# danieleschmidt/spin-torque-rl-gym

Hardware: AMD Instinct MI355X
Metric: env_steps_per_sec (higher is better)
Workload: dtype f64

## Files before the change

### spin-torque-rl-gym_amd/csrc/stg_kernels.hpp

```cpp
#pragma once
#include "../../include/spintorque_hip.h"
#include "stg_launch_plan.hpp"
#include "stg_physics.hpp"

#include <hip/hip_runtime.h>

#include <type_traits>

using namespace stg;

struct alignas(16) EnvRec {
    double m[3];
    double tgt[3];
    double etot;
    uint32_t stepw;
    uint32_t rng;
};
static_assert(sizeof(EnvRec) == 64, "state record size");
constexpr uint32_t STG_DONE_BIT = 0x80000000u;

struct StateView {
    EnvRec* rec;
};

// ... 400 lines not shown
        } else {
            write_obs(a.final_obs + ko * 12 * N, N, i, m, tgt, row, a.c, step, etot, J, T);
        }
    }
    if (do_reset) {
        device_reset_draw(a.c.seed, env_id, rng, a.c, true, true, m, tgt);
        etot = 0.0; step = 0; done = false;
        J = 0.0; T = 0.0;
    }
    if (wr) {
        if (a.records) {
            write_record((char*)a.obs + ko * N * STG_RECORD_BYTES, i, m, tgt, row, a.c, step, etot, J, T, (float)reward,
                         (is_success ? 1u : 0u) | (truncated ? 0x100u : 0u) | ((uint32_t)st << 16));
        } else {
            write_obs(a.obs + ko * 12 * N, N, i, m, tgt, row, a.c, step, etot, J, T);
            a.reward[ko * N + i] = (float)reward;
            a.term[ko * N + i] = is_success ? 1 : 0;
            a.trunc[ko * N + i] = truncated ? 1 : 0;
        }
        if (a.reward64) a.reward64[ko * N + i] = reward;
        if (a.energy) a.energy[ko * N + i] = energy;
        if (a.status) a.status[ko * N + i] = st;
    }
}

constexpr int REFILL_STRIPES = 64;
constexpr int REFILL_CURSOR_STRIDE = 16;

template <bool THERMAL, bool MULTI, bool AXIS_Z, typename AT, bool IDS>
__device__ __forceinline__ void refill_wave(const StepArgs& a, int64_t w, int64_t nw, int64_t blk0, int64_t nblk_q, int lane, const double* s_tab,
                                            unsigned long long& c_steps, unsigned long long& c_sub, unsigned long long& c_noop) {
    const int64_t N = a.N;
    const int64_t tiles = (N + TILE_ENVS - 1) / TILE_ENVS;
    if (w == 0 && lane < REFILL_STRIPES) a.refill_cursor_next[lane * REFILL_CURSOR_STRIDE] = 0ull;
    const AT* act = (const AT*)a.actions;
    const Recorder norec{};
    const LlgsEnergyK noek{};
    const Dp5Tab tb = make_dp5_tab();
    InlineNormals ns;

    int64_t i = 0, o = 0;
    bool has_env = false;
    double J = 0.0, T = 0.0;
    V3 e_tgt{0.0, 0.0, 1.0};
    double e_etot = 0.0;
    int32_t e_step = 0;
    uint32_t e_rng = 0;
    bool e_skip = false;
    const double* row = a.ctab;
    LlgsK k = load_llgs(row);
    LlgsLane L;
    L.active = false; L.idle = true; L.rejected = false; L.attempts = 0; L.npts = 0;
    L.y = L.f = L.m0 = V3{0.0, 0.0, 1.0};
    L.t = L.T = L.h_abs = L.min_step = L.bJ = L.bpJ = 0.0;
    V3 out_m{0.0, 0.0, 1.0};

    auto take = [&](int64_t p, bool want) {
        const int64_t idx = blk0 + (p >> 6);
        const bool valid_blk = want && (p >> 6) < nblk_q;
        const int64_t slot = (valid_blk ? refill_slot_base(idx, tiles) : 0) + (p & 63);
        const bool valid = valid_blk && slot < N;
        if (!valid) return;
        if constexpr (IDS) {
            o = a.perm ? (int64_t)a.perm[slot] : slot;
            const uint32_t id = a.ids[o];
            if ((int64_t)id >= a.n_state) { write_bad_id(a, o); return; }
            i = (int64_t)id;
        } else {
            i = a.perm ? (int64_t)a.perm[slot] : slot;
        }
        V3 m;
        bool done;
        load_state(a.s, i, m, e_tgt, e_etot, e_step, e_rng, done);
        const uint32_t rng = e_rng;
        if (a.perm) {
            typedef typename std::conditional<std::is_same<AT, double>::value, double2, float2>::type AT2;
            const AT2 aa = ((const AT2*)a.act_sorted)[slot];
            parse_action<AT>(aa.x, aa.y, a.c.max_current, a.c.max_duration, J, T);
        } else {
            const int64_t p = IDS ? o : i;
            parse_action<AT>(act[p], act[N + p], a.c.max_current, a.c.max_duration, J, T);
        }
        if (MULTI) {
            const int c = (int)a.cls[i];
            row = s_tab + (c < a.ncls ? c : 0) * C_COUNT;
            k = load_llgs(row);
        }
        const RngKey rk{a.c.seed, (uint64_t)(a.env_id0 + i), rng};
        e_skip = a.c.skip_done && done;
        llgs_lane_begin<THERMAL, false, AXIS_Z>(L, out_m, m, J, T, k, row[C_BETA], row[C_BETAP], a.c.rtol, a.c.atol, a.c.max_step, rk,
                                                norec, noek, ns, !e_skip);
        has_env = true;
    };
    auto finish = [&]() {
        const SolveOut so = llgs_lane_finish<false>(L, out_m, norec, noek, ns);
        V3 m = L.m0, tgt = e_tgt;
        double etot = e_etot;
        int32_t step = e_step;
        uint32_t rng = e_rng;
        bool done = e_skip;
        env_step_tail(a, IDS ? o : i, 0, true, true, !e_skip, row, (uint64_t)(a.env_id0 + i), m, tgt, etot, step, rng, done, J, T, so, c_steps, c_sub, c_noop);
        store_state(a.s, i, m, tgt, etot, step, rng, done);
        has_env = false;
        L.active = false;
    };

    take(w * 64 + lane, true);
    const int64_t n_rest = nblk_q > nw ? nblk_q - nw : 0;
    static_assert(REFILL_STRIPES == 64, "one lane per stripe when a wavefront looks for a stripe that still has entries");
    int stripe = (int)(w % REFILL_STRIPES);
    bool queue_open = true;
    int64_t loc_q = 0, loc_end = 0;
    int loc_stripe = 0, full_streak = 0;
    bool more = n_rest > 0;
    const int check = a.refill_check > 0 ? a.refill_check : 1;
    for (;;) {
        LlgsMasks M = llgs_masks_open(L);
        for (int c = 0; c < check; ++c) {
            llgs_lane_gate<false>(L, M, (int32_t)a.c.max_attempts);
            if (M.active == 0ull) break;
            V3 z2{0.0, 0.0, 0.0}, z3{0.0, 0.0, 0.0};
            llgs_lane_attempt<THERMAL, false, AXIS_Z, false>(L, M, 0, out_m, k, tb, a.c.rtol, a.c.atol, a.c.max_step, norec, noek, ns, z2, z3);
        }
        llgs_masks_close(L, M);
        const bool fin = has_env && !L.active;
        if (__ballot(fin) != 0ull || (more && __ballot(!has_env) != 0ull)) {
            if (fin) finish();
            const unsigned long long takers = __ballot(!has_env);
            if (more && takers != 0ull) {
                const int n_take = (int)__builtin_popcountll(takers), first = (int)__builtin_ctzll(takers);
                const int rank = (int)__builtin_popcountll(takers & ((1ull << lane) - 1ull));
                const int64_t avail = loc_end - loc_q;
                const int need_new = n_take > avail ? (int)(n_take - avail) : 0;
                int64_t new_q = 0;
                const int new_stripe = stripe;
                if (need_new > 0 && queue_open) {
                    const int reserve = (takers == ~0ull && full_streak >= 1) ? 4 * 64 : need_new;
                    unsigned long long base = 0;
                    if (lane == first) base = atomicAdd(a.refill_cursor + stripe * REFILL_CURSOR_STRIDE, (unsigned long long)reserve);
                    base = (unsigned long long)__shfl((long long)base, first);
                    new_q = (int64_t)base;
                    const int64_t stripe_end = ((n_rest - stripe + REFILL_STRIPES - 1) / REFILL_STRIPES) * 64;
                    int64_t new_end = new_q + reserve;
                    if (new_end >= stripe_end) {
                        new_end = stripe_end;
                        const int64_t end_l = ((n_rest - lane + REFILL_STRIPES - 1) / REFILL_STRIPES) * 64;
                        const unsigned long long cur_l = __hip_atomic_load(a.refill_cursor + lane * REFILL_CURSOR_STRIDE, __ATOMIC_RELAXED, __HIP_MEMORY_SCOPE_AGENT);
                        unsigned long long open_s = __ballot((int64_t)cur_l < end_l);
                        open_s &= ~(1ull << stripe);
                        if (open_s == 0ull) queue_open = false;
                        else {
                            const unsigned long long after = stripe == 63 ? 0ull : (open_s >> (stripe + 1)) << (stripe + 1);
                            stripe = (int)__builtin_ctzll(after != 0ull ? after : open_s);
                        }
                    }
                    const bool from_old = rank < avail;
                    const int64_t q = from_old ? loc_q + rank : new_q + (rank - avail);
                    const int st = from_old ? loc_stripe : new_stripe;
                    const int64_t r = (q >> 6) * REFILL_STRIPES + st;
                    take((nw + r) * 64 + (q & 63), !has_env && r < n_rest && (from_old || q < new_end));
                    loc_q = new_q + need_new < new_end ? new_q + need_new : new_end;
                    loc_end = new_end;
                    loc_stripe = new_stripe;
                } else {
                    const int64_t q = loc_q + rank;
                    const int64_t r = (q >> 6) * REFILL_STRIPES + loc_stripe;
                    take((nw + r) * 64 + (q & 63), !has_env && q < loc_end && r < n_rest);
                    loc_q = loc_q + n_take < loc_end ? loc_q + n_take : loc_end;
                }
                more = queue_open || loc_q < loc_end;
                full_streak = takers == ~0ull ? full_streak + 1 : 0;
            }
        }
        if (__ballot(has_env) == 0ull && !more) break;
    }
// ... 230 lines not shown
```

### spin-torque-rl-gym_amd/csrc/stg_physics.hpp

```cpp
#pragma once

#include <hip/hip_runtime.h>
#include <stdint.h>
#include <type_traits>

#include "stg_minstep.hpp"

namespace stg {

enum ClassConst : int {
    C_EX = 0, C_EY, C_EZ,
    C_HK,
    C_MS,
    C_ALPHA,
    C_GEFF,
    C_POL,
    C_MSV,
    C_HS_SIMPLE,
    C_RX, C_RY, C_RZ,
    C_DX, C_DY, C_DZ,
    C_HEX,
    C_BETA, C_BETAP,
    C_GAMMA,
    C_HS_LLGS,
// ... 29 lines not shown
    r[C_HS_SIMPLE] = sqrt(2 * p.damping * 1.38e-23 * temperature / (mu0 * p.ms * p.volume * gamma));
    r[C_RX] = p.easy_axis[0]; r[C_RY] = p.easy_axis[1]; r[C_RZ] = p.easy_axis[2];
    r[C_DX] = -p.ms * p.demag[0]; r[C_DY] = -p.ms * p.demag[1]; r[C_DZ] = -p.ms * p.demag[2];
    r[C_HEX] = p.a_ex > 0 ? (2 * p.a_ex / (mu0 * p.ms)) * 0.1 : 0.0;
    r[C_BETA] = p.polarization * gamma / (2 * p.ms * p.volume);
    r[C_BETAP] = 0.1 * r[C_BETA];
    r[C_GAMMA] = gamma;
    r[C_HS_LLGS] = sqrt(2 * p.damping * 1.380649e-23 * temperature / (gamma * mu0 * p.ms * p.volume));
    r[C_KUV] = p.ku * p.volume;
    r[C_EDEMAG] = 0.5 * mu0 * (p.ms * p.ms) * p.volume;
    r[C_NX] = p.demag[0]; r[C_NY] = p.demag[1]; r[C_NZ] = p.demag[2];
    r[C_AREA] = p.area; r[C_RP] = p.r_p; r[C_RAP] = p.r_ap;
    r[C_TMR] = (p.r_ap - p.r_p) / p.r_p;
    const double rn = sqrt((p.ref_m[0] * p.ref_m[0] + p.ref_m[1] * p.ref_m[1]) + p.ref_m[2] * p.ref_m[2]);
    r[C_REFX] = p.ref_m[0] / rn; r[C_REFY] = p.ref_m[1] / rn; r[C_REFZ] = p.ref_m[2] / rn;
    r[C_RSERIES] = p.r_series;
    r[C_DEVTYPE] = (double)p.dev_type;
    r[C_VALID] = p.params_valid ? 1.0 : 0.0;
    r[C_SOT_DL] = p.sot_tau_dl; r[C_SOT_FL] = p.sot_tau_fl;
    r[C_SIGX] = p.sot_sigma[0]; r[C_SIGY] = p.sot_sigma[1]; r[C_SIGZ] = p.sot_sigma[2];
    r[C_KU] = p.ku;
    r[C_VCMA_XI] = p.vcma_xi;
    r[C_VCMA_TD2] = p.vcma_td * p.vcma_td;
    r[C_VCMA_VBD] = p.vcma_vbd;
    r[C_MU0MS] = mu0 * p.ms;
}

struct V3 {
    double x, y, z;
};

__device__ __forceinline__ double mul_x(double a, double b) {
#pragma clang fp contract(off)
    const double r = a * b;
    return r;
}
__device__ __forceinline__ double add_x(double a, double b) {
#pragma clang fp contract(off)
    const double r = a + b;
    return r;
}
__device__ __forceinline__ double sub_x(double a, double b) {
#pragma clang fp contract(off)
    const double r = a - b;
    return r;
}

__device__ __forceinline__ double rsqrt_fast(double s) {
    const double y = __builtin_amdgcn_rsq(s);
    const double e = __builtin_fma(-(s * y), y, 1.0);
    return __builtin_fma(y * e, __builtin_fma(0.375, e, 0.5), y);
}

__device__ __forceinline__ double vgpr_const(double c) {
    asm volatile("" : "+v"(c));
    return c;
}

__device__ __forceinline__ double fmax_abs(double a, double b) {
    double r;
    asm("v_max_f64 %0, |%1|, |%2|" : "=v"(r) : "v"(a), "v"(b));
    return r;
}

__device__ __forceinline__ void commit_step(unsigned long long mask, double& d0, double s0, double& d1, double s1, double& d2, double s2,
                                            double& d3, double s3, double& d4, double s4, double& d5, double s5, double& d6, double s6,
                                            double& min_step, double& h, double unit) {
    unsigned long long saved;
    int e;
    asm("s_and_saveexec_b64 %[sv], %[m]\n\t"
        "v_mov_b64 %[d0], %[s0]\n\t"
        "v_mov_b64 %[d1], %[s1]\n\t"
        "v_mov_b64 %[d2], %[s2]\n\t"
        "v_mov_b64 %[d3], %[s3]\n\t"
        "v_mov_b64 %[d4], %[s4]\n\t"
        "v_mov_b64 %[d5], %[s5]\n\t"
        "v_mov_b64 %[d6], %[s6]\n\t"
        "v_frexp_exp_i32_f64 %[e], %[s0]\n\t"
        "v_max_i32 %[e], %[fl], %[e]\n\t"
        "v_ldexp_f64 %[ms], %[u], %[e]\n\t"
        "v_max_f64 %[h], %[h], %[ms]\n\t"
        "s_mov_b64 exec, %[sv]"
        : [d0] "+v"(d0), [d1] "+v"(d1), [d2] "+v"(d2), [d3] "+v"(d3), [d4] "+v"(d4), [d5] "+v"(d5), [d6] "+v"(d6), [ms] "+v"(min_step),
          [h] "+v"(h), [e] "=&v"(e), [sv] "=&s"(saved)
        : [s0] "v"(s0), [s1] "v"(s1), [s2] "v"(s2), [s3] "v"(s3), [s4] "v"(s4), [s5] "v"(s5), [s6] "v"(s6), [u] "v"(unit), [m] "s"(mask),
          [fl] "n"(MIN_STEP_EXP_FLOOR)
        : "scc");
}

__device__ __forceinline__ double rcp_fast(double x) {
    const double y = __builtin_amdgcn_rcp(x);
    return __builtin_fma(y, __builtin_fma(-x, y, 1.0), y);
}

__device__ __forceinline__ double inv_tenth_root(double e2) {
    const double y = (double)__builtin_amdgcn_exp2f(-0.1f * __builtin_amdgcn_logf((float)e2));
    const double y2 = y * y, y4 = y2 * y2, y8 = y4 * y4;
    const double e = __builtin_fma(-e2, y8 * y2, 1.0);
    return __builtin_fma(y * e, __builtin_fma(0.055, e, 0.1), y);
}

__device__ __forceinline__ double fifth_root(double x) {
    int e;
    const double mant = frexp(x, &e);
    const double t = -0.2 * ((double)e + (double)__builtin_amdgcn_logf((float)mant));
    const double ti = rint(t);
    double r = ldexp((double)__builtin_amdgcn_exp2f((float)(t - ti)), (int)ti);
    const double r2 = r * r, r4 = r2 * r2;
    const double err = __builtin_fma(-x, r4 * r, 1.0);
    r = __builtin_fma(r * err, __builtin_fma(0.12, err, 0.2), r);
    const double q2 = r * r;
    return x * (q2 * q2);
}

__device__ __forceinline__ V3 cross(const V3& a, const V3& b) {
#pragma clang fp contract(off)
    return V3{__builtin_fma(a.y, b.z, -(a.z * b.y)), __builtin_fma(a.z, b.x, -(a.x * b.z)), __builtin_fma(a.x, b.y, -(a.y * b.x))};
}
__device__ __forceinline__ double dot(const V3& a, const V3& b) {
#pragma clang fp contract(off)
    return __builtin_fma(a.z, b.z, __builtin_fma(a.y, b.y, a.x * b.x));
}
__device__ __forceinline__ V3 scale3(double c, const V3& z) {
#pragma clang fp contract(off)
    return V3{c * z.x, c * z.y, c * z.z};
}
__device__ __forceinline__ bool finite3(const V3& a) { return isfinite(a.x) && isfinite(a.y) && isfinite(a.z); }

__device__ __forceinline__ void philox4x32_10(uint32_t c0, uint32_t c1, uint32_t c2, uint32_t c3, uint32_t k0,
                                              uint32_t k1, uint32_t (&out)[4]) {
#pragma unroll
    for (int r = 0; r < 10; ++r) {
        const uint32_t hi0 = __umulhi(0xD2511F53u, c0), lo0 = 0xD2511F53u * c0;
        const uint32_t hi1 = __umulhi(0xCD9E8D57u, c2), lo1 = 0xCD9E8D57u * c2;
        const uint32_t n0 = hi1 ^ c1 ^ k0, n2 = hi0 ^ c3 ^ k1;
        c0 = n0; c1 = lo1; c2 = n2; c3 = lo0;
        k0 += 0x9E3779B9u; k1 += 0xBB67AE85u;
    }
    out[0] = c0; out[1] = c1; out[2] = c2; out[3] = c3;
}

struct NormalStream {
    uint32_t s0, s1, s2, s3;
    float carry;
    __device__ __forceinline__ void init(uint64_t seed, uint64_t env_id, uint32_t env_step, uint32_t tag) {
        uint32_t r[4];
        philox4x32_10((uint32_t)env_id, (uint32_t)(env_id >> 32), env_step, tag, (uint32_t)seed, (uint32_t)(seed >> 32), r);
        s0 = r[0]; s1 = r[1]; s2 = r[2]; s3 = r[3] | 1u;
        carry = 0.0f;
    }
    __device__ __forceinline__ uint32_t next() {
        const uint32_t result = s0 + s3;
// ... 2 lines not shown
        s3 = (s3 << 11) | (s3 >> 21);
        return result;
    }
    __device__ __forceinline__ float uniform() {
        return __uint_as_float(__builtin_amdgcn_alignbit(0x7fu, next(), 9u)) - 0.99999994f;
    }
    typedef float f32x2 __attribute__((ext_vector_type(2)));
    __device__ __forceinline__ void pair(float& a, float& b) {
        float t, c, s_;
        pair_head(t, c, s_);
        finish_pair(t, c, s_, a, b);
    }
    __device__ __forceinline__ void pair_head(float& t, float& c, float& s_) {
        f32x2 u{__uint_as_float(__builtin_amdgcn_alignbit(0x7fu, next(), 9u)), __uint_as_float(__builtin_amdgcn_alignbit(0x7fu, next(), 9u))};
        u = u - f32x2{0.99999994f, 0.99999994f};
        t = -1.3862943611198906f * __builtin_amdgcn_logf(u.x);
        c = __builtin_amdgcn_cosf(u.y);
        s_ = __builtin_amdgcn_sinf(u.y);
    }
    static __device__ __forceinline__ void finish_pair(float t, float c, float s_, float& a, float& b) {
        const float r = __builtin_amdgcn_sqrtf(t);
        const f32x2 cs = f32x2{c, s_} * f32x2{r, r};
        a = cs.x;
        b = cs.y;
    }
    __device__ __forceinline__ V3 draw3_even() {
        float a, b, c, d;
        pair(a, b);
        pair(c, d);
        carry = d;
        return V3{(double)a, (double)b, (double)c};
    }
    __device__ __forceinline__ V3 draw3_odd() {
        float a, b;
        pair(a, b);
        return V3{(double)carry, (double)a, (double)b};
    }
};

struct RngKey {
    uint64_t seed, env_id;
    uint32_t env_step;
};

struct InlineNormals {
    static constexpr bool kShared = false, kScaled = false;
    NormalStream ns;
    __device__ __forceinline__ void begin(const RngKey& rk) { ns.init(rk.seed, rk.env_id, rk.env_step, 0u); }
    __device__ __forceinline__ V3 draw(bool even) { return even ? ns.draw3_even() : ns.draw3_odd(); }
    static constexpr bool broken = false;
    __device__ __forceinline__ void peek() {}
    __device__ __forceinline__ bool chunk_end(bool lane_continues) { return lane_continues; }
    __device__ __forceinline__ bool chunk_end_wave(bool mine) { return mine; }
};

constexpr int SHARED_SUBS_RK4 = 2;
constexpr int SHARED_SUBS3 = 4 * SHARED_SUBS_RK4;
constexpr int SHARED_CHUNK_FIXED = 12 * SHARED_SUBS_RK4;
constexpr int SHARED_CHUNK_RK45 = 18;
constexpr int PC_STOP = 1 << 30;
constexpr int PC_SPIN_CAP = 1 << 22;

typedef __attribute__((address_space(3))) int lds_int;
__device__ __forceinline__ volatile lds_int* lds_flag(const int* p) { return (volatile lds_int*)p; }

template <int WGW>
__device__ __forceinline__ bool any_flag(volatile lds_int* f) {
    int v = f[0];
#pragma unroll
    for (int j = 1; j < WGW; ++j) v |= f[j];
    return v != 0;
}
__device__ __forceinline__ int pc_load(const int* p) {
    return __builtin_amdgcn_readfirstlane(__hip_atomic_load(p, __ATOMIC_ACQUIRE, __HIP_MEMORY_SCOPE_WORKGROUP));
}
__device__ __forceinline__ void pc_store(int* p, int v) {
    __hip_atomic_store(p, v, __ATOMIC_RELEASE, __HIP_MEMORY_SCOPE_WORKGROUP);
}

template <typename T, bool SCALED, int DEPTH, bool BARRIER>
struct SharedNormalsT {
    static constexpr int CHUNK = SCALED ? SHARED_CHUNK_RK45 : SHARED_CHUNK_FIXED;
    static_assert(!BARRIER || DEPTH == 2, "the barrier form runs the producer exactly one chunk ahead");
    static constexpr bool kShared = true, kScaled = SCALED;
    const T* buf;
    int* hs;
    int lane, it, idx, seen;
    bool broken;
    static constexpr bool kToggle = BARRIER && SCALED;
    int slot_el, flag_el;
    __device__ __forceinline__ void begin(const RngKey&) {
        it = 0; idx = 0; seen = 1; broken = false;
        if (kToggle) {
            static_assert(((CHUNK * 64) & 63) == 0, "the slot bit and the lane bits are disjoint");
            slot_el = lane; flag_el = 0;
            asm volatile("" : "+v"(slot_el), "+v"(flag_el));
        }
    }
    __device__ __forceinline__ V3 draw(bool) {
        const T* b = kToggle ? buf + slot_el + idx * 64 : buf + ((it & (DEPTH - 1)) * CHUNK + idx) * 64 + lane;
        idx += 3;
        return V3{(double)b[0], (double)b[64], (double)b[128]};
    }
    __device__ __forceinline__ void peek() {
        if (!BARRIER) seen = __hip_atomic_load(hs, __ATOMIC_RELAXED, __HIP_MEMORY_SCOPE_WORKGROUP);
    }
    __device__ __forceinline__ bool chunk_end(bool lane_continues) { return chunk_end_wave(__ballot(lane_continues) != 0ull); }
    __device__ __forceinline__ bool chunk_end_wave(bool mine) {
        if (BARRIER) {
            lds_flag(hs)[kToggle ? flag_el : (it & 1)] = mine ? 1 : 0;
            if (kToggle) { flag_el ^= 1; slot_el ^= CHUNK * 64; }
            __syncthreads();
            ++it;
            idx = 0;
            return mine;
        }
        ++it;
        idx = 0;
        pc_store(hs + 1, it | (mine ? 0 : PC_STOP));
        int have = __builtin_amdgcn_readfirstlane(seen);
        if (__builtin_expect(mine && have <= it, 0)) {
            int spins = 0;
#pragma unroll 1
            do {
                if (spins) __builtin_amdgcn_s_sleep(1);
                have = pc_load(hs);
            } while (have <= it && ++spins <= PC_SPIN_CAP);
            broken = broken || have <= it;
        }
        seen = have;
        __builtin_amdgcn_fence(__ATOMIC_ACQUIRE, "workgroup");
        return mine && !broken;
    }
};

template <typename T, bool SCALED, int DEPTH, bool BARRIER>
__device__ __forceinline__ void produce_normals(T* buf, int* hs, int lane, const RngKey& rk, int n_first, int n_chunk, double c) {
    NormalStream ns;
    ns.init(rk.seed, rk.env_id, rk.env_step, 0u);
    bool even = true;
    auto fill = [&](int slot, int count) {
        T* b = buf + (slot * (SCALED ? SHARED_CHUNK_RK45 : SHARED_CHUNK_FIXED)) * 64 + lane;
        for (int j = 0; j < count; j += 3) {
            V3 z = even ? ns.draw3_even() : ns.draw3_odd();
            if (SCALED) z = scale3(c, z);
            even = !even;
            b[(j + 0) * 64] = (T)z.x; b[(j + 1) * 64] = (T)z.y; b[(j + 2) * 64] = (T)z.z;
        }
    };
    fill(0, n_first);
    if (!BARRIER) pc_store(hs, 1);
    __syncthreads();
    if (BARRIER) {
        for (int k = 1;; ++k) {
            fill(k & 1, n_chunk);
            __syncthreads();
            if (lds_flag(hs)[(k - 1) & 1] == 0) return;
        }
    }
    for (int k = 1;; ++k) {
        int v = pc_load(hs + 1);
#pragma unroll 1
        for (int spins = 0; (v & (PC_STOP - 1)) < k - DEPTH + 1 && !(v & PC_STOP); ++spins) {
            if (spins > PC_SPIN_CAP) return;
            __builtin_amdgcn_s_sleep(1);
            v = pc_load(hs + 1);
        }
        if (v & PC_STOP) return;
        fill(k & (DEPTH - 1), n_chunk);
        pc_store(hs, k + 1);
    }
}

struct SimpleK {
    V3 e;
    double ghk;
    double gdm;
    double alpha;
    double ghs;
};
__device__ __forceinline__ SimpleK make_simple(const V3& e, double hk, double ms, double alpha, double geff, double hs) {
#pragma clang fp contract(off)
    return SimpleK{e, -geff * hk, geff * ms, alpha, -geff * hs};
}
struct LlgsK {
// ... 245 lines not shown
    const double inv = rsqrt_fast(ss);
    V3 m{y.x * inv, y.y * inv, y.z * inv};
    if (CHECKED) {
        const bool unit = ss > 1e-24;
        if (__builtin_expect(__ballot(!unit) != 0ull, 0)) m = V3{unit ? m.x : 0.0, unit ? m.y : 0.0, unit ? m.z : 1.0};
    }
    if (AXIS_Z) {
        const double u = __builtin_fma(k.gz, m.z, bpJ);
        const double w = __builtin_fma(k.agz, m.z, bJ);
        if (!THERMAL) {
            const double c = m.z * w;
            return V3{__builtin_fma(m.x, c, m.y * u), __builtin_fma(m.y, c, -(m.x * u)), __builtin_fma(m.z, c, -w)};
        }
        const double uz = ht.z + u;
        const V3 W{k.alpha * ht.x, k.alpha * ht.y, __builtin_fma(k.alpha, ht.z, w)};
        const double s = dot(m, W);
        return V3{__builtin_fma(m.x, s, __builtin_fma(m.y, uz, __builtin_fma(-m.z, ht.y, -W.x))),
                  __builtin_fma(m.y, s, __builtin_fma(m.z, ht.x, __builtin_fma(-m.x, uz, -W.y))),
                  __builtin_fma(m.z, s, __builtin_fma(m.x, ht.y, __builtin_fma(-m.y, ht.x, -W.z)))};
    }
    const double c = k.ghk * dot(m, k.r);
    V3 g{(c * k.r.x + k.gd.x * m.x) + k.ghex * m.x, (c * k.r.y + k.gd.y * m.y) + k.ghex * m.y,
         (c * k.r.z + k.gd.z * m.z) + k.ghex * m.z};
    if (THERMAL) g = V3{g.x + ht.x, g.y + ht.y, g.z + ht.z};
    const V3 U{g.x, g.y, g.z + bpJ};
    const V3 W{k.alpha * g.x, k.alpha * g.y, __builtin_fma(k.alpha, g.z, bJ)};
    const double s = dot(m, W);
    return V3{__builtin_fma(m.x, s, __builtin_fma(m.y, U.z, __builtin_fma(-m.z, U.y, -W.x))),
              __builtin_fma(m.y, s, __builtin_fma(m.z, U.x, __builtin_fma(-m.x, U.z, -W.y))),
              __builtin_fma(m.z, s, __builtin_fma(m.x, U.y, __builtin_fma(-m.y, U.x, -W.z)))};
}

struct LlgsEnergyK {
    double kuv, edemag;
    V3 r, nfac;
};
__device__ __forceinline__ double llgs_energy(const V3& m, const LlgsEnergyK& k) {
    const double ct = dot(m, k.r);
    return -k.kuv * (ct * ct) + k.edemag * (k.nfac.x * (m.x * m.x) + k.nfac.y * (m.y * m.y) + k.nfac.z * (m.z * m.z));
}

__device__ __forceinline__ double llgs_torque_norms(const V3& m, double bJ, double bpJ) {
#pragma clang fp contract(off)
    const V3 mxp{m.y, -m.x, 0.0};
    const V3 mm = cross(m, mxp);
    const V3 a{bJ * mm.x, bJ * mm.y, bJ * mm.z}, b{bpJ * mxp.x, bpJ * mxp.y, bpJ * mxp.z};
    return sqrt((a.x * a.x + a.y * a.y) + a.z * a.z) + sqrt((b.x * b.x + b.y * b.y) + b.z * b.z);
}

__device__ __forceinline__ double rms3(const V3& a) { return sqrt(dot(a, a)) / 1.7320508075688772; }

struct Dp5Tab {
    double A51, A52, A53, A54, A61, A62, A63, A64, A65, E1, E3, E4, E5, E6, E7;
    double ms_unit;
};
__device__ __forceinline__ Dp5Tab make_dp5_tab() {
    Dp5Tab t;
    t.A51 = vgpr_const(19372.0 / 6561); t.A52 = vgpr_const(-25360.0 / 2187); t.A53 = vgpr_const(64448.0 / 6561); t.A54 = vgpr_const(-212.0 / 729);
    t.A61 = vgpr_const(9017.0 / 3168); t.A62 = vgpr_const(-355.0 / 33); t.A63 = vgpr_const(46732.0 / 5247); t.A64 = vgpr_const(49.0 / 176);
    t.A65 = vgpr_const(-5103.0 / 18656);
    t.E1 = vgpr_const(-71.0 / 57600); t.E3 = vgpr_const(71.0 / 16695); t.E4 = vgpr_const(-71.0 / 1920); t.E5 = vgpr_const(17253.0 / 339200);
    t.E6 = vgpr_const(-22.0 / 525); t.E7 = vgpr_const(1.0 / 40);
    t.ms_unit = vgpr_const(MIN_STEP_UNIT);
    return t;
}

struct LlgsLane {
    V3 y, f;
    V3 m0;
    double t, T, h_abs, min_step;
    double bJ, bpJ;
    int32_t attempts;
    int32_t npts;
    bool idle;
    bool rejected, active;
};

typedef unsigned long long lanemask;
struct LlgsMasks {
    lanemask active, pacc;
};
__device__ __forceinline__ bool lane_in(lanemask m) { return __builtin_amdgcn_inverse_ballot_w64(m); }
__device__ __forceinline__ LlgsMasks llgs_masks_open(const LlgsLane& L) { return LlgsMasks{__ballot(L.active), __ballot(!L.rejected)}; }
__device__ __forceinline__ void llgs_masks_close(LlgsLane& L, const LlgsMasks& M) {
    L.active = lane_in(M.active);
    L.rejected = !lane_in(M.pacc);
}

template <bool RECORD>
__device__ __forceinline__ void llgs_lane_emit(LlgsLane& L, V3& out_m, const Recorder& rec, const LlgsEnergyK& ek) {
    const double inv = rsqrt_fast(dot(L.y, L.y));
    out_m = V3{L.y.x * inv, L.y.y * inv, L.y.z * inv};
    if (RECORD) rec.put(L.npts, L.t, out_m, rec.e ? llgs_energy(out_m, ek) : 0.0, rec.tq ? llgs_torque_norms(out_m, L.bJ, L.bpJ) : 0.0);
    ++L.npts;
}

template <bool THERMAL, bool AXIS_Z, bool CHECKED = true>
__device__ __forceinline__ V3 llgs_fun(const LlgsLane& L, const LlgsK& k, const V3& y, const V3& ht, bool on) {
    return llgs_rhs<THERMAL, AXIS_Z, CHECKED>(y, k, on ? L.bJ : 0.0, on ? L.bpJ : 0.0, ht);
}
template <bool THERMAL, class NSRC>
__device__ __forceinline__ V3 llgs_draw(NSRC& ns, const LlgsK& k, bool even) {
    if (!THERMAL) return V3{0.0, 0.0, 0.0};
    return NSRC::kScaled ? ns.draw(even) : scale3(k.ghs, ns.draw(even));
}

template <bool THERMAL, bool RECORD, bool AXIS_Z, class NSRC>
__device__ __forceinline__ void llgs_lane_begin(LlgsLane& L, V3& out_m, const V3& m0, double J, double T, const LlgsK& k, double beta,
                                                double betap, double rtol, double atol, double max_step, const RngKey& rk,
                                                const Recorder& rec, const LlgsEnergyK& ek, NSRC& ns, bool enabled) {
    const bool useJ = !(fabs(J) < 1e-12);
    L.bJ = useJ ? beta * J : 0.0;
    L.bpJ = useJ ? betap * J : 0.0;
    L.m0 = m0;
    L.T = T;
    if (THERMAL) ns.begin(rk);
    const double n0 = rsqrt_fast(dot(m0, m0));
    L.y = V3{m0.x * n0, m0.y * n0, m0.z * n0};
    L.t = 0.0;
    L.npts = 0;
    if (RECORD) llgs_lane_emit<RECORD>(L, out_m, rec, ek); else ++L.npts;
    L.f = llgs_fun<THERMAL, AXIS_Z>(L, k, L.y, llgs_draw<THERMAL>(ns, k, true), true);
    double h_abs;
    {
        const V3& y = L.y;
        const V3& f = L.f;
        const V3 sc{atol + fabs(y.x) * rtol, atol + fabs(y.y) * rtol, atol + fabs(y.z) * rtol};
        const V3 isc{rcp_fast(sc.x), rcp_fast(sc.y), rcp_fast(sc.z)};
        const double d0 = rms3(V3{y.x * isc.x, y.y * isc.y, y.z * isc.z});
        const double d1 = rms3(V3{f.x * isc.x, f.y * isc.y, f.z * isc.z});
        double h0 = (d0 < 1e-5 || d1 < 1e-5) ? 1e-6 : (0.01 * d0) * rcp_fast(d1);
        h0 = fmin(h0, T);
        const V3 y1{y.x + h0 * f.x, y.y + h0 * f.y, y.z + h0 * f.z};
        const V3 f1 = llgs_fun<THERMAL, AXIS_Z>(L, k, y1, llgs_draw<THERMAL>(ns, k, false), true);
        const double d2 = rms3(V3{(f1.x - f.x) * isc.x, (f1.y - f.y) * isc.y, (f1.z - f.z) * isc.z}) * rcp_fast(h0);
        const double h1 = (d1 <= 1e-15 && d2 <= 1e-15) ? fmax(1e-6, h0 * 1e-3) : fifth_root(0.01 * rcp_fast(fmax(d1, d2)));
        h_abs = fmin(fmin(100.0 * h0, h1), fmin(T, max_step));
    }
    L.rejected = false;
    L.attempts = 0;
    L.min_step = min_step_at(L.t);
    L.h_abs = h_abs > max_step ? max_step : (h_abs < L.min_step ? L.min_step : h_abs);
    L.active = enabled && (L.t != T);
    L.idle = !L.active;
}

template <bool UNIFORM_IT>
__device__ __forceinline__ void llgs_lane_gate(const LlgsLane& L, LlgsMasks& M, int32_t max_attempts) {
    lanemask stop = __ballot(L.h_abs < L.min_step);
    if (!UNIFORM_IT) stop |= __ballot(L.attempts >= max_attempts);
    M.active &= ~stop;
}

template <bool THERMAL, bool RECORD, bool AXIS_Z, bool UNIFORM_IT, class NSRC>
__device__ __forceinline__ void llgs_lane_attempt(LlgsLane& L, LlgsMasks& M, int32_t it, V3& out_m, const LlgsK& k, const Dp5Tab& tb, double rtol,
                                                  double atol, double max_step, const Recorder& rec, const LlgsEnergyK& ek, NSRC& ns, V3 z2, V3 z3) {
    constexpr double A21 = 1.0 / 5;
    constexpr double A31 = 3.0 / 40, A32 = 9.0 / 40;
    constexpr double A41 = 44.0 / 45, A42 = -56.0 / 15, A43 = 32.0 / 9;
    constexpr double B1 = 35.0 / 384, B3 = 500.0 / 1113, B4 = 125.0 / 192, B5 = -2187.0 / 6784, B6 = 11.0 / 84;
    const double A51 = tb.A51, A52 = tb.A52, A53 = tb.A53, A54 = tb.A54, A61 = tb.A61, A62 = tb.A62, A63 = tb.A63, A64 = tb.A64, A65 = tb.A65;
    const double E1 = tb.E1, E3 = tb.E3, E4 = tb.E4, E5 = tb.E5, E6 = tb.E6, E7 = tb.E7;
    const double T = L.T;
    const bool active = lane_in(M.active);
    const V3 y = L.y;
    const double t = L.t;
    auto fun = [&](const V3& yy, const V3& ht, bool on) -> V3 { return llgs_fun<THERMAL, AXIS_Z, false>(L, k, yy, ht, on); };
    auto draw = [&](bool even) -> V3 { return llgs_draw<THERMAL>(ns, k, even); };
    if (UNIFORM_IT) L.attempts = active ? it + 1 : L.attempts; else L.attempts += active ? 1 : 0;
    const double t_new = fmin(add_x(t, L.h_abs), T);
    const double h = sub_x(t_new, t);
    const double h_try = fabs(h);
    const bool on_end = add_x(t, h) <= T;
    const V3 k1 = L.f;
    if (THERMAL && !NSRC::kShared) { z2 = draw(true); z3 = draw(false); }
    const V3 k2 = fun(V3{y.x + (k1.x * A21) * h, y.y + (k1.y * A21) * h, y.z + (k1.z * A21) * h}, z2, true);
    const V3 z4 = draw(true);
    const V3 k3 = fun(V3{y.x + (k1.x * A31 + k2.x * A32) * h, y.y + (k1.y * A31 + k2.y * A32) * h,
                         y.z + (k1.z * A31 + k2.z * A32) * h}, z3, true);
    const V3 z5 = draw(false);
    const V3 k4 = fun(V3{y.x + (k1.x * A41 + k2.x * A42 + k3.x * A43) * h, y.y + (k1.y * A41 + k2.y * A42 + k3.y * A43) * h,
                         y.z + (k1.z * A41 + k2.z * A42 + k3.z * A43) * h}, z4, true);
    const V3 z6 = draw(true);
    const V3 k5 = fun(V3{y.x + (k1.x * A51 + k2.x * A52 + k3.x * A53 + k4.x * A54) * h,
                         y.y + (k1.y * A51 + k2.y * A52 + k3.y * A53 + k4.y * A54) * h,
                         y.z + (k1.z * A51 + k2.z * A52 + k3.z * A53 + k4.z * A54) * h}, z5, true);
    if (THERMAL) ns.peek();
    const V3 z7 = draw(false);
    const V3 k6 = fun(V3{y.x + (k1.x * A61 + k2.x * A62 + k3.x * A63 + k4.x * A64 + k5.x * A65) * h,
                         y.y + (k1.y * A61 + k2.y * A62 + k3.y * A63 + k4.y * A64 + k5.y * A65) * h,
                         y.z + (k1.z * A61 + k2.z * A62 + k3.z * A63 + k4.z * A64 + k5.z * A65) * h}, z6, on_end);
    const V3 y_new{y.x + h * (k1.x * B1 + k3.x * B3 + k4.x * B4 + k5.x * B5 + k6.x * B6),
                   y.y + h * (k1.y * B1 + k3.y * B3 + k4.y * B4 + k5.y * B5 + k6.y * B6),
                   y.z + h * (k1.z * B1 + k3.z * B3 + k4.z * B4 + k5.z * B5 + k6.z * B6)};
    const V3 f_new = fun(y_new, z7, on_end);
    const V3 ev{(k1.x * E1 + k3.x * E3 + k4.x * E4 + k5.x * E5 + k6.x * E6 + f_new.x * E7) * h,
                (k1.y * E1 + k3.y * E3 + k4.y * E4 + k5.y * E5 + k6.y * E6 + f_new.y * E7) * h,
                (k1.z * E1 + k3.z * E3 + k4.z * E4 + k5.z * E5 + k6.z * E6 + f_new.z * E7) * h};
    const V3 sc{atol + fmax_abs(y.x, y_new.x) * rtol, atol + fmax_abs(y.y, y_new.y) * rtol, atol + fmax_abs(y.z, y_new.z) * rtol};
    const V3 q{ev.x * rcp_fast(sc.x), ev.y * rcp_fast(sc.y), ev.z * rcp_fast(sc.z)};
    const double err2 = dot(q, q) * (1.0 / 3.0);
    const double err = err2;
    const lanemask accm = M.active & __ballot(err < 1.0);
    const bool acc = lane_in(accm);
    const double r9 = 0.9 * inv_tenth_root(err);
    const double fa = fmin(lane_in(M.pacc) ? 10.0 : 1.0, r9);
    const double fr = fmax(0.2, r9);
    double h_next = fmin(h_try * (acc ? fa : fr), max_step);
    commit_step(accm, L.t, t_new, L.y.x, y_new.x, L.y.y, y_new.y, L.y.z, y_new.z, L.f.x, f_new.x, L.f.y, f_new.y, L.f.z, f_new.z,
                L.min_step, h_next, tb.ms_unit);
    L.h_abs = h_next;
    if (RECORD) { if (acc) llgs_lane_emit<RECORD>(L, out_m, rec, ek); } else L.npts += acc ? 1 : 0;
    M.pacc = accm;
    M.active &= __ballot(L.t != T);
}

template <bool RECORD, class NSRC>
__device__ __forceinline__ SolveOut llgs_lane_finish(LlgsLane& L, V3& out_m, const Recorder& rec, const LlgsEnergyK& ek, const NSRC& ns) {
    SolveOut o{L.m0, 0, 0, 0, false};
    if (!RECORD) { llgs_lane_emit<RECORD>(L, out_m, rec, ek); --L.npts; }
    o.m = out_m;
    o.n = L.npts - 1;
    o.work = L.attempts;
    const bool ok = L.idle || L.t == L.T;
    o.ok = ok && !ns.broken;
    if (!ok) o.m = L.m0;
    return o;
}

template <bool THERMAL, bool RECORD, bool AXIS_Z, class NSRC>
__device__ __forceinline__ SolveOut llgs_solve(const V3& m0, double J, double T, const LlgsK& k, double beta,
                                               double betap, double rtol, double atol, double max_step,
                                               int64_t max_attempts, const RngKey& rk, const Recorder& rec,
                                               const LlgsEnergyK& ek, NSRC& ns, bool enabled) {
    const Dp5Tab tb = make_dp5_tab();
    const V3 zero{0.0, 0.0, 0.0};
    LlgsLane L;
    V3 out_m = m0;
    llgs_lane_begin<THERMAL, RECORD, AXIS_Z>(L, out_m, m0, J, T, k, beta, betap, rtol, atol, max_step, rk, rec, ek, ns, enabled);
    LlgsMasks M = llgs_masks_open(L);
    atol = vgpr_const(atol);
    const int32_t budget = (int32_t)max_attempts;
    int32_t it = 0;
    bool wave_go = true;
    if (NSRC::kShared) wave_go = ns.chunk_end_wave(M.active != 0ull);
    if (wave_go)
    for (;;) {
      V3 z2 = zero, z3 = zero;
      if (THERMAL && NSRC::kShared) { z2 = llgs_draw<THERMAL>(ns, k, true); z3 = llgs_draw<THERMAL>(ns, k, false); }
      llgs_lane_gate<true>(L, M, budget);
      if (!NSRC::kShared && M.active == 0ull) break;
      llgs_lane_attempt<THERMAL, RECORD, AXIS_Z, true>(L, M, it, out_m, k, tb, rtol, atol, max_step, rec, ek, ns, z2, z3);
      ++it;
      const bool go = it < budget;
      if (NSRC::kShared) { if (!ns.chunk_end_wave(go && M.active != 0ull)) break; }
      else if (!go) break;
    }
    llgs_masks_close(L, M);
    return llgs_lane_finish<RECORD>(L, out_m, rec, ek, ns);
}

__device__ __forceinline__ double resistance(const V3& m_in, int dev_type, double r_p, double r_ap, double tmr,
                                             const V3& ref, double r_series) {
#pragma clang fp contract(off)
    if (dev_type == 0) {
        const double inv = rsqrt_fast(dot(m_in, m_in));
        const V3 m{m_in.x * inv, m_in.y * inv, m_in.z * inv};
        const double r = r_p * (1.0 + tmr * (1.0 - dot(m, ref)) * 0.5);
        return fmax(r, r_p * 0.5);
    }
    double r = r_p + (r_ap - r_p) * (1.0 - dot(m_in, ref)) * 0.5;
    if (dev_type == 1) r = r + r_series;
    return fmax(r, 1.0);
}

template <typename AT>
__device__ __forceinline__ void parse_action(AT a0, AT a1, double max_current, double max_duration, double& J, double& T) {
    const AT cmax = (AT)1e8, dmin = (AT)1e-12, dmax = (AT)1e-6;
    if (!isnan(a0)) a0 = a0 < -cmax ? -cmax : (a0 > cmax ? cmax : a0);
    if (!isnan(a1)) a1 = a1 < dmin ? dmin : (a1 > dmax ? dmax : a1);
    if (isnan(a0) || isnan(a1) || isinf(a0) || isinf(a1)) { a0 = (AT)0; a1 = dmin; }
    const double j = (double)a0, t = (double)a1;
    J = j < -max_current ? -max_current : (j > max_current ? max_current : j);
    T = t < 1e-12 ? 1e-12 : (t > max_duration ? max_duration : t);
}

__device__ __forceinline__ float obs_cast(double v) {
    const float f = (float)v;
    return isnan(f) ? 0.0f : (isinf(f) ? (f > 0 ? 1e6f : -1e6f) : f);
}

}
```

Before: 43.31 million.

## Hoist min-step floor check out of the per-attempt commit and batch thermal noise loads

Removes the per-attempt min-step recomputation (frexp/ldexp/max) from the commit asm. It is replaced by a precomputed conservative floor (the min step at the end time T) and a rarely taken branch that recomputes the exact min step only when h drops below that floor. It also batches the shared noise draws two at a time behind scheduling barriers, moves several constants into VGPRs, and folds the loop-exit logic into scalar asm with byte-offset LDS addressing. This cuts per-attempt ALU work and scalar overhead but changes control flow and could alter rare clamping semantics.

Result: faster. 44.21 million, median of 6 (+2.1%).

```diff
diff --git a/spin-torque-rl-gym_amd/csrc/stg_kernels.hpp b/spin-torque-rl-gym_amd/csrc/stg_kernels.hpp
--- a/spin-torque-rl-gym_amd/csrc/stg_kernels.hpp
+++ b/spin-torque-rl-gym_amd/csrc/stg_kernels.hpp
@@ -476,7 +476,7 @@
     LlgsLane L;
     L.active = false; L.idle = true; L.rejected = false; L.attempts = 0; L.npts = 0;
     L.y = L.f = L.m0 = V3{0.0, 0.0, 1.0};
-    L.t = L.T = L.h_abs = L.min_step = L.bJ = L.bpJ = 0.0;
+    L.t = L.T = L.h_abs = L.h_floor = L.bJ = L.bpJ = 0.0;
     V3 out_m{0.0, 0.0, 1.0};
 
     auto take = [&](int64_t p, bool want) {
@@ -544,7 +544,7 @@
             llgs_lane_gate<false>(L, M, (int32_t)a.c.max_attempts);
             if (M.active == 0ull) break;
             V3 z2{0.0, 0.0, 0.0}, z3{0.0, 0.0, 0.0};
-            llgs_lane_attempt<THERMAL, false, AXIS_Z, false>(L, M, 0, out_m, k, tb, a.c.rtol, a.c.atol, a.c.max_step, norec, noek, ns, z2, z3);
+            llgs_lane_attempt<THERMAL, false, AXIS_Z, false>(L, M, out_m, k, tb, a.c.rtol, a.c.atol, a.c.max_step, norec, noek, ns, z2, z3);
         }
         llgs_masks_close(L, M);
         const bool fin = has_env && !L.active;
diff --git a/spin-torque-rl-gym_amd/csrc/stg_physics.hpp b/spin-torque-rl-gym_amd/csrc/stg_physics.hpp
--- a/spin-torque-rl-gym_amd/csrc/stg_physics.hpp
+++ b/spin-torque-rl-gym_amd/csrc/stg_physics.hpp
@@ -105,6 +105,10 @@
     return __builtin_fma(y * e, __builtin_fma(0.375, e, 0.5), y);
 }
 
+__device__ __forceinline__ void batch_ready(double at, double a0, double a1, double a2, double b0, double b1, double b2) {
+    asm volatile("" : : "v"(at), "v"(a0), "v"(a1), "v"(a2), "v"(b0), "v"(b1), "v"(b2));
+}
+
 __device__ __forceinline__ double vgpr_const(double c) {
     asm volatile("" : "+v"(c));
     return c;
@@ -117,10 +121,8 @@
 }
 
 __device__ __forceinline__ void commit_step(unsigned long long mask, double& d0, double s0, double& d1, double s1, double& d2, double s2,
-                                            double& d3, double s3, double& d4, double s4, double& d5, double s5, double& d6, double s6,
-                                            double& min_step, double& h, double unit) {
+                                            double& d3, double s3, double& d4, double s4, double& d5, double s5, double& d6, double s6) {
     unsigned long long saved;
-    int e;
     asm("s_and_saveexec_b64 %[sv], %[m]\n\t"
         "v_mov_b64 %[d0], %[s0]\n\t"
         "v_mov_b64 %[d1], %[s1]\n\t"
@@ -129,15 +131,9 @@
         "v_mov_b64 %[d4], %[s4]\n\t"
         "v_mov_b64 %[d5], %[s5]\n\t"
         "v_mov_b64 %[d6], %[s6]\n\t"
-        "v_frexp_exp_i32_f64 %[e], %[s0]\n\t"
-        "v_max_i32 %[e], %[fl], %[e]\n\t"
-        "v_ldexp_f64 %[ms], %[u], %[e]\n\t"
-        "v_max_f64 %[h], %[h], %[ms]\n\t"
         "s_mov_b64 exec, %[sv]"
-        : [d0] "+v"(d0), [d1] "+v"(d1), [d2] "+v"(d2), [d3] "+v"(d3), [d4] "+v"(d4), [d5] "+v"(d5), [d6] "+v"(d6), [ms] "+v"(min_step),
-          [h] "+v"(h), [e] "=&v"(e), [sv] "=&s"(saved)
-        : [s0] "v"(s0), [s1] "v"(s1), [s2] "v"(s2), [s3] "v"(s3), [s4] "v"(s4), [s5] "v"(s5), [s6] "v"(s6), [u] "v"(unit), [m] "s"(mask),
-          [fl] "n"(MIN_STEP_EXP_FLOOR)
+        : [d0] "+v"(d0), [d1] "+v"(d1), [d2] "+v"(d2), [d3] "+v"(d3), [d4] "+v"(d4), [d5] "+v"(d5), [d6] "+v"(d6), [sv] "=&s"(saved)
+        : [s0] "v"(s0), [s1] "v"(s1), [s2] "v"(s2), [s3] "v"(s3), [s4] "v"(s4), [s5] "v"(s5), [s6] "v"(s6), [m] "s"(mask)
         : "scc");
 }
 
@@ -146,11 +142,11 @@
     return __builtin_fma(y, __builtin_fma(-x, y, 1.0), y);
 }
 
-__device__ __forceinline__ double inv_tenth_root(double e2) {
+__device__ __forceinline__ double inv_tenth_root(double e2, double tenth = 0.1) {
     const double y = (double)__builtin_amdgcn_exp2f(-0.1f * __builtin_amdgcn_logf((float)e2));
     const double y2 = y * y, y4 = y2 * y2, y8 = y4 * y4;
     const double e = __builtin_fma(-e2, y8 * y2, 1.0);
-    return __builtin_fma(y * e, __builtin_fma(0.055, e, 0.1), y);
+    return __builtin_fma(y * e, __builtin_fma(0.055, e, tenth), y);
 }
 
 __device__ __forceinline__ double fifth_root(double x) {
@@ -259,6 +255,7 @@
     __device__ __forceinline__ void peek() {}
     __device__ __forceinline__ bool chunk_end(bool lane_continues) { return lane_continues; }
     __device__ __forceinline__ bool chunk_end_wave(bool mine) { return mine; }
+    __device__ __forceinline__ int32_t chunk_end_go(int32_t go) { return go; }
 };
 
 constexpr int SHARED_SUBS_RK4 = 2;
@@ -295,17 +292,17 @@
     int lane, it, idx, seen;
     bool broken;
     static constexpr bool kToggle = BARRIER && SCALED;
-    int slot_el, flag_el;
+    int slot_b, flag_b;
     __device__ __forceinline__ void begin(const RngKey&) {
         it = 0; idx = 0; seen = 1; broken = false;
         if (kToggle) {
             static_assert(((CHUNK * 64) & 63) == 0, "the slot bit and the lane bits are disjoint");
-            slot_el = lane; flag_el = 0;
-            asm volatile("" : "+v"(slot_el), "+v"(flag_el));
+            slot_b = lane * (int)sizeof(T); flag_b = 0;
+            asm volatile("" : "+v"(slot_b), "+v"(flag_b));
         }
     }
     __device__ __forceinline__ V3 draw(bool) {
-        const T* b = kToggle ? buf + slot_el + idx * 64 : buf + ((it & (DEPTH - 1)) * CHUNK + idx) * 64 + lane;
+        const T* b = kToggle ? (const T*)((const char*)buf + slot_b) + idx * 64 : buf + ((it & (DEPTH - 1)) * CHUNK + idx) * 64 + lane;
         idx += 3;
         return V3{(double)b[0], (double)b[64], (double)b[128]};
     }
@@ -313,14 +310,20 @@
         if (!BARRIER) seen = __hip_atomic_load(hs, __ATOMIC_RELAXED, __HIP_MEMORY_SCOPE_WORKGROUP);
     }
     __device__ __forceinline__ bool chunk_end(bool lane_continues) { return chunk_end_wave(__ballot(lane_continues) != 0ull); }
-    __device__ __forceinline__ bool chunk_end_wave(bool mine) {
+    __device__ __forceinline__ bool chunk_end_wave(bool mine) { return chunk_end_go(mine ? 1 : 0) != 0; }
+    __device__ __forceinline__ int32_t chunk_end_go(int32_t go) {
+        const bool mine = go != 0;
         if (BARRIER) {
-            lds_flag(hs)[kToggle ? flag_el : (it & 1)] = mine ? 1 : 0;
-            if (kToggle) { flag_el ^= 1; slot_el ^= CHUNK * 64; }
+            if (kToggle) {
+                *(volatile lds_int*)((volatile __attribute__((address_space(3))) char*)lds_flag(hs) + flag_b) = go;
+                flag_b ^= (int)sizeof(int); slot_b ^= CHUNK * 64 * (int)sizeof(T);
+            } else {
+                lds_flag(hs)[it & 1] = go;
+            }
             __syncthreads();
             ++it;
             idx = 0;
-            return mine;
+            return go;
         }
         ++it;
         idx = 0;
@@ -337,7 +340,7 @@
         }
         seen = have;
         __builtin_amdgcn_fence(__ATOMIC_ACQUIRE, "workgroup");
-        return mine && !broken;
+        return (mine && !broken) ? 1 : 0;
     }
 };
 
@@ -689,7 +692,7 @@
 
 struct Dp5Tab {
     double A51, A52, A53, A54, A61, A62, A63, A64, A65, E1, E3, E4, E5, E6, E7;
-    double ms_unit;
+    double B4, third, c09, tenth;
 };
 __device__ __forceinline__ Dp5Tab make_dp5_tab() {
     Dp5Tab t;
@@ -698,14 +701,15 @@
     t.A65 = vgpr_const(-5103.0 / 18656);
     t.E1 = vgpr_const(-71.0 / 57600); t.E3 = vgpr_const(71.0 / 16695); t.E4 = vgpr_const(-71.0 / 1920); t.E5 = vgpr_const(17253.0 / 339200);
     t.E6 = vgpr_const(-22.0 / 525); t.E7 = vgpr_const(1.0 / 40);
-    t.ms_unit = vgpr_const(MIN_STEP_UNIT);
+    t.B4 = vgpr_const(125.0 / 192); t.third = vgpr_const(1.0 / 3.0); t.c09 = vgpr_const(0.9); t.tenth = vgpr_const(0.1);
     return t;
 }
 
 struct LlgsLane {
     V3 y, f;
     V3 m0;
-    double t, T, h_abs, min_step;
+    double t, T, h_abs;
+    double h_floor;
     double bJ, bpJ;
     int32_t attempts;
     int32_t npts;
@@ -715,10 +719,12 @@
 
 typedef unsigned long long lanemask;
 struct LlgsMasks {
-    lanemask active, pacc;
+    lanemask active, pacc, low;
 };
 __device__ __forceinline__ bool lane_in(lanemask m) { return __builtin_amdgcn_inverse_ballot_w64(m); }
-__device__ __forceinline__ LlgsMasks llgs_masks_open(const LlgsLane& L) { return LlgsMasks{__ballot(L.active), __ballot(!L.rejected)}; }
+__device__ __forceinline__ LlgsMasks llgs_masks_open(const LlgsLane& L) {
+    return LlgsMasks{__ballot(L.active), __ballot(!L.rejected), __ballot(L.h_abs < L.h_floor)};
+}
 __device__ __forceinline__ void llgs_masks_close(LlgsLane& L, const LlgsMasks& M) {
     L.active = lane_in(M.active);
     L.rejected = !lane_in(M.pacc);
@@ -776,26 +782,44 @@
     }
     L.rejected = false;
     L.attempts = 0;
-    L.min_step = min_step_at(L.t);
-    L.h_abs = h_abs > max_step ? max_step : (h_abs < L.min_step ? L.min_step : h_abs);
+    const double min_step = min_step_at(L.t);
+    L.h_abs = h_abs > max_step ? max_step : (h_abs < min_step ? min_step : h_abs);
+    L.h_floor = isfinite(T) ? min_step_at(T) : __builtin_inf();
     L.active = enabled && (L.t != T);
     L.idle = !L.active;
 }
 
 template <bool UNIFORM_IT>
-__device__ __forceinline__ void llgs_lane_gate(const LlgsLane& L, LlgsMasks& M, int32_t max_attempts) {
-    lanemask stop = __ballot(L.h_abs < L.min_step);
-    if (!UNIFORM_IT) stop |= __ballot(L.attempts >= max_attempts);
-    M.active &= ~stop;
+__device__ __forceinline__ void llgs_lane_gate(LlgsLane& L, LlgsMasks& M, int32_t max_attempts) {
+    if (__builtin_expect((M.low & M.active) != 0ull, 0)) {
+        const double min_step = min_step_at(L.t);
+        if (lane_in(M.pacc)) L.h_abs = L.h_abs < min_step ? min_step : L.h_abs;
+        M.active &= ~__ballot(L.h_abs < min_step);
+    }
+    if (!UNIFORM_IT) M.active &= ~__ballot(L.attempts >= max_attempts);
+}
+
+__device__ __forceinline__ int32_t attempt_loop_next(lanemask& active, lanemask not_arrived, int32_t& it, int32_t budget) {
+    int32_t go;
+    asm("s_add_i32 %[it], %[it], 1\n\t"
+        "s_and_b64 %[act], %[act], %[na]\n\t"
+        "s_cselect_b32 %[go], %[bud], 0\n\t"
+        "s_cmp_lt_i32 %[it], %[go]\n\t"
+        "s_cselect_b32 %[go], 1, 0"
+        : [act] "+s"(active), [it] "+s"(it), [go] "=&s"(go)
+        : [na] "s"(not_arrived), [bud] "s"(budget)
+        : "scc");
+    return go;
 }
 
 template <bool THERMAL, bool RECORD, bool AXIS_Z, bool UNIFORM_IT, class NSRC>
-__device__ __forceinline__ void llgs_lane_attempt(LlgsLane& L, LlgsMasks& M, int32_t it, V3& out_m, const LlgsK& k, const Dp5Tab& tb, double rtol,
+__device__ __forceinline__ void llgs_lane_attempt(LlgsLane& L, LlgsMasks& M, V3& out_m, const LlgsK& k, const Dp5Tab& tb, double rtol,
                                                   double atol, double max_step, const Recorder& rec, const LlgsEnergyK& ek, NSRC& ns, V3 z2, V3 z3) {
     constexpr double A21 = 1.0 / 5;
     constexpr double A31 = 3.0 / 40, A32 = 9.0 / 40;
     constexpr double A41 = 44.0 / 45, A42 = -56.0 / 15, A43 = 32.0 / 9;
-    constexpr double B1 = 35.0 / 384, B3 = 500.0 / 1113, B4 = 125.0 / 192, B5 = -2187.0 / 6784, B6 = 11.0 / 84;
+    constexpr double B1 = 35.0 / 384, B3 = 500.0 / 1113, B5 = -2187.0 / 6784, B6 = 11.0 / 84;
+    const double B4 = tb.B4;
     const double A51 = tb.A51, A52 = tb.A52, A53 = tb.A53, A54 = tb.A54, A61 = tb.A61, A62 = tb.A62, A63 = tb.A63, A64 = tb.A64, A65 = tb.A65;
     const double E1 = tb.E1, E3 = tb.E3, E4 = tb.E4, E5 = tb.E5, E6 = tb.E6, E7 = tb.E7;
     const double T = L.T;
@@ -804,29 +828,38 @@
     const double t = L.t;
     auto fun = [&](const V3& yy, const V3& ht, bool on) -> V3 { return llgs_fun<THERMAL, AXIS_Z, false>(L, k, yy, ht, on); };
     auto draw = [&](bool even) -> V3 { return llgs_draw<THERMAL>(ns, k, even); };
-    if (UNIFORM_IT) L.attempts = active ? it + 1 : L.attempts; else L.attempts += active ? 1 : 0;
+    L.attempts += active ? 1 : 0;
     const double t_new = fmin(add_x(t, L.h_abs), T);
     const double h = sub_x(t_new, t);
     const double h_try = fabs(h);
     const bool on_end = add_x(t, h) <= T;
     const V3 k1 = L.f;
+    constexpr bool BATCH = THERMAL && NSRC::kShared;
     if (THERMAL && !NSRC::kShared) { z2 = draw(true); z3 = draw(false); }
-    const V3 k2 = fun(V3{y.x + (k1.x * A21) * h, y.y + (k1.y * A21) * h, y.z + (k1.z * A21) * h}, z2, true);
-    const V3 z4 = draw(true);
+    V3 y2{y.x + (k1.x * A21) * h, y.y + (k1.y * A21) * h, y.z + (k1.z * A21) * h};
+    if (BATCH) batch_ready(y2.z, z2.x, z2.y, z2.z, z3.x, z3.y, z3.z);
+    const V3 k2 = fun(y2, z2, true);
+    V3 z4 = draw(true), z5{0.0, 0.0, 0.0};
+    if (BATCH) { z5 = draw(false); __builtin_amdgcn_sched_barrier(0); }
     const V3 k3 = fun(V3{y.x + (k1.x * A31 + k2.x * A32) * h, y.y + (k1.y * A31 + k2.y * A32) * h,
                          y.z + (k1.z * A31 + k2.z * A32) * h}, z3, true);
-    const V3 z5 = draw(false);
-    const V3 k4 = fun(V3{y.x + (k1.x * A41 + k2.x * A42 + k3.x * A43) * h, y.y + (k1.y * A41 + k2.y * A42 + k3.y * A43) * h,
-                         y.z + (k1.z * A41 + k2.z * A42 + k3.z * A43) * h}, z4, true);
-    const V3 z6 = draw(true);
+    if (!BATCH) z5 = draw(false);
+    V3 y4{y.x + (k1.x * A41 + k2.x * A42 + k3.x * A43) * h, y.y + (k1.y * A41 + k2.y * A42 + k3.y * A43) * h,
+          y.z + (k1.z * A41 + k2.z * A42 + k3.z * A43) * h};
+    if (BATCH) batch_ready(y4.z, z4.x, z4.y, z4.z, z5.x, z5.y, z5.z);
+    const V3 k4 = fun(y4, z4, true);
+    V3 z6 = draw(true), z7{0.0, 0.0, 0.0};
+    if (BATCH) { z7 = draw(false); __builtin_amdgcn_sched_barrier(0); }
     const V3 k5 = fun(V3{y.x + (k1.x * A51 + k2.x * A52 + k3.x * A53 + k4.x * A54) * h,
                          y.y + (k1.y * A51 + k2.y * A52 + k3.y * A53 + k4.y * A54) * h,
                          y.z + (k1.z * A51 + k2.z * A52 + k3.z * A53 + k4.z * A54) * h}, z5, true);
     if (THERMAL) ns.peek();
-    const V3 z7 = draw(false);
-    const V3 k6 = fun(V3{y.x + (k1.x * A61 + k2.x * A62 + k3.x * A63 + k4.x * A64 + k5.x * A65) * h,
-                         y.y + (k1.y * A61 + k2.y * A62 + k3.y * A63 + k4.y * A64 + k5.y * A65) * h,
-                         y.z + (k1.z * A61 + k2.z * A62 + k3.z * A63 + k4.z * A64 + k5.z * A65) * h}, z6, on_end);
+    if (!BATCH) z7 = draw(false);
+    V3 y6{y.x + (k1.x * A61 + k2.x * A62 + k3.x * A63 + k4.x * A64 + k5.x * A65) * h,
+          y.y + (k1.y * A61 + k2.y * A62 + k3.y * A63 + k4.y * A64 + k5.y * A65) * h,
+          y.z + (k1.z * A61 + k2.z * A62 + k3.z * A63 + k4.z * A64 + k5.z * A65) * h};
+    if (BATCH) batch_ready(y6.z, z6.x, z6.y, z6.z, z7.x, z7.y, z7.z);
+    const V3 k6 = fun(y6, z6, on_end);
     const V3 y_new{y.x + h * (k1.x * B1 + k3.x * B3 + k4.x * B4 + k5.x * B5 + k6.x * B6),
                    y.y + h * (k1.y * B1 + k3.y * B3 + k4.y * B4 + k5.y * B5 + k6.y * B6),
                    y.z + h * (k1.z * B1 + k3.z * B3 + k4.z * B4 + k5.z * B5 + k6.z * B6)};
@@ -836,20 +869,20 @@
                 (k1.z * E1 + k3.z * E3 + k4.z * E4 + k5.z * E5 + k6.z * E6 + f_new.z * E7) * h};
     const V3 sc{atol + fmax_abs(y.x, y_new.x) * rtol, atol + fmax_abs(y.y, y_new.y) * rtol, atol + fmax_abs(y.z, y_new.z) * rtol};
     const V3 q{ev.x * rcp_fast(sc.x), ev.y * rcp_fast(sc.y), ev.z * rcp_fast(sc.z)};
-    const double err2 = dot(q, q) * (1.0 / 3.0);
+    const double err2 = dot(q, q) * tb.third;
     const double err = err2;
     const lanemask accm = M.active & __ballot(err < 1.0);
     const bool acc = lane_in(accm);
-    const double r9 = 0.9 * inv_tenth_root(err);
+    const double r9 = tb.c09 * inv_tenth_root(err, tb.tenth);
     const double fa = fmin(lane_in(M.pacc) ? 10.0 : 1.0, r9);
     const double fr = fmax(0.2, r9);
     double h_next = fmin(h_try * (acc ? fa : fr), max_step);
-    commit_step(accm, L.t, t_new, L.y.x, y_new.x, L.y.y, y_new.y, L.y.z, y_new.z, L.f.x, f_new.x, L.f.y, f_new.y, L.f.z, f_new.z,
-                L.min_step, h_next, tb.ms_unit);
+    M.low = __ballot(h_next < L.h_floor);
     L.h_abs = h_next;
+    commit_step(accm, L.t, t_new, L.y.x, y_new.x, L.y.y, y_new.y, L.y.z, y_new.z, L.f.x, f_new.x, L.f.y, f_new.y, L.f.z, f_new.z);
     if (RECORD) { if (acc) llgs_lane_emit<RECORD>(L, out_m, rec, ek); } else L.npts += acc ? 1 : 0;
     M.pacc = accm;
-    M.active &= __ballot(L.t != T);
+    if (!UNIFORM_IT) M.active &= __ballot(L.t != T);
 }
 
 template <bool RECORD, class NSRC>
@@ -877,21 +910,18 @@
     llgs_lane_begin<THERMAL, RECORD, AXIS_Z>(L, out_m, m0, J, T, k, beta, betap, rtol, atol, max_step, rk, rec, ek, ns, enabled);
     LlgsMasks M = llgs_masks_open(L);
     atol = vgpr_const(atol);
-    const int32_t budget = (int32_t)max_attempts;
+    int32_t budget = (int32_t)max_attempts;
+    asm volatile("" : "+s"(budget));
     int32_t it = 0;
-    bool wave_go = true;
-    if (NSRC::kShared) wave_go = ns.chunk_end_wave(M.active != 0ull);
+    bool wave_go = M.active != 0ull;
+    if (NSRC::kShared) wave_go = ns.chunk_end_wave(wave_go);
     if (wave_go)
     for (;;) {
       V3 z2 = zero, z3 = zero;
       if (THERMAL && NSRC::kShared) { z2 = llgs_draw<THERMAL>(ns, k, true); z3 = llgs_draw<THERMAL>(ns, k, false); }
       llgs_lane_gate<true>(L, M, budget);
-      if (!NSRC::kShared && M.active == 0ull) break;
-      llgs_lane_attempt<THERMAL, RECORD, AXIS_Z, true>(L, M, it, out_m, k, tb, rtol, atol, max_step, rec, ek, ns, z2, z3);
-      ++it;
-      const bool go = it < budget;
-      if (NSRC::kShared) { if (!ns.chunk_end_wave(go && M.active != 0ull)) break; }
-      else if (!go) break;
+      llgs_lane_attempt<THERMAL, RECORD, AXIS_Z, true>(L, M, out_m, k, tb, rtol, atol, max_step, rec, ek, ns, z2, z3);
+      if (!ns.chunk_end_go(attempt_loop_next(M.active, __ballot(L.t != L.T), it, budget))) break;
     }
     llgs_masks_close(L, M);
     return llgs_lane_finish<RECORD>(L, out_m, rec, ek, ns);
```
